# shadowk29/cusumtools

Hardware: NVIDIA B200
Metric: Msamples/s filtered+CUSUM-segmented (higher is better)
Workload: dtype f32

## Files before the change

cusumtools_b200/csrc/ct_detect.cu:

```cuda
#include "ct_common.cuh"
#include "cusumtools_b200.h"

namespace {

constexpr int kRun = 4096;
constexpr int kRunWords = kRun / 32;
constexpr int kDetWarps = 8;

struct RunSummary {
    unsigned first_last;
    unsigned ns0;
    unsigned ne0;
    unsigned pad;
};

__device__ __forceinline__ unsigned automaton_word(unsigned A, unsigned B, unsigned& c) {
    unsigned P = ~(A | B);
    unsigned long long X = (unsigned long long)(A | P), Y = (unsigned long long)A;
    unsigned long long sum = X + Y + c;
    unsigned long long cin = sum ^ X ^ Y;
    unsigned I = (unsigned)(cin >> 1);
    c = I >> 31;
    return I;
}
// ... 95 lines not shown
        A[2 * k] = A[2 * k + 1] = a; B[2 * k] = B[2 * k + 1] = b;
        mixed[k] = mix;
    }
#pragma unroll
    for (int k = 0; k < 2; ++k) {
        unsigned todo = __ballot_sync(CT_FULL, mixed[k]);
        while (todo) {
            const int src = __ffs(todo) - 1;
            todo &= todo - 1;
            const long long p0 = base + (2 * src + k) * 64 + lane, p1 = p0 + 32;
            const float v0 = p0 < n ? sgn * y[p0] : te, v1 = p1 < n ? sgn * y[p1] : te;
            const unsigned a0 = __ballot_sync(CT_FULL, v0 < ts), b0 = __ballot_sync(CT_FULL, v0 > te);
            const unsigned a1 = __ballot_sync(CT_FULL, v1 < ts), b1 = __ballot_sync(CT_FULL, v1 > te);
            if (lane == src) { A[2 * k] = a0; B[2 * k] = b0; A[2 * k + 1] = a1; B[2 * k + 1] = b1; }
        }
    }
    uint4* mout = reinterpret_cast<uint4*>(masks + run * kRunWords + 4 * lane);
    mout[0] = make_uint4(A[0], B[0], A[1], B[1]);
    mout[1] = make_uint4(A[2], B[2], A[3], B[3]);
    unsigned lastIn = 0, firstIn = 0, any = 0;
#pragma unroll
    for (int w = 0; w < 4; ++w) {
        const unsigned nz = A[w] | B[w];
        if (nz) {
            if (!any) firstIn = (A[w] >> (__ffs(nz) - 1)) & 1u;
            lastIn = (A[w] >> (31 - __clz(nz))) & 1u;
            any = 1;
        }
    }
    const unsigned nzmask = __ballot_sync(CT_FULL, any != 0);
    const unsigned lastmask = __ballot_sync(CT_FULL, lastIn != 0);
    const unsigned firstmask = __ballot_sync(CT_FULL, firstIn != 0);
    const unsigned lower = nzmask & ((1u << lane) - 1u);
    unsigned c = lower ? ((lastmask >> (31 - __clz(lower))) & 1u) : 0u;
    unsigned ns = 0, ne = 0;
#pragma unroll
    for (int w = 0; w < 4; ++w) {
        const unsigned cprev = c;
        const unsigned I = automaton_word(A[w], B[w], c);
        const unsigned prev = (I << 1) | cprev;
        ns += __popc(I & ~prev);
        ne += __popc(~I & prev);
    }
#pragma unroll
    for (int o = 16; o > 0; o >>= 1) { ns += __shfl_xor_sync(CT_FULL, ns, o); ne += __shfl_xor_sync(CT_FULL, ne, o); }
    if (lane == 0) {
        unsigned first = 0, last = 0;
        if (nzmask) {
            first = ((firstmask >> (__ffs(nzmask) - 1)) & 1u) ? 1u : 2u;
            last = ((lastmask >> (31 - __clz(nzmask))) & 1u) ? 1u : 2u;
        }
        RunSummary s; s.first_last = first | (last << 2); s.ns0 = ns; s.ne0 = ne; s.pad = 0;
        summ[run] = s;
    }
}

__device__ __forceinline__ void adjusted(const RunSummary& s, unsigned st, unsigned& a, unsigned& b) {
    const unsigned f = s.first_last & 3;
    a = s.ns0; b = s.ne0;
    if (st == 1) { if (f == 1) a -= 1; else if (f == 2) b += 1; }
}
constexpr int kGroup = 64;
__global__ void ct_detect_scan_groups(const RunSummary* __restrict__ summ, long long nruns,
                                      RunSummary* __restrict__ gsum, long long ngroups) {
    const long long g = (long long)blockIdx.x * blockDim.x + threadIdx.x;
    if (g >= ngroups) return;
    const long long r0 = g * kGroup, r1 = (r0 + kGroup < nruns) ? r0 + kGroup : nruns;
    unsigned st = 2, first = 0, last = 0, ns = 0, ne = 0;
    for (long long r = r0; r < r1; ++r) {
        const RunSummary s = summ[r];
        unsigned a, b; adjusted(s, st, a, b);
        ns += a; ne += b;
        const unsigned f = s.first_last & 3, l = (s.first_last >> 2) & 3;
        if (!first) first = f;
        if (l) { last = l; st = l; }
    }
    RunSummary o; o.first_last = first | (last << 2); o.ns0 = ns; o.ne0 = ne; o.pad = 0;
    gsum[g] = o;
}
__global__ void ct_detect_scan_expand(const RunSummary* __restrict__ summ, long long nruns,
                                      const uint4* __restrict__ ginfo, const unsigned long long* __restrict__ goffs,
                                      long long ngroups, uint4* __restrict__ runinfo,
                                      unsigned long long* __restrict__ offs) {
    const long long g = (long long)blockIdx.x * blockDim.x + threadIdx.x;
    if (g >= ngroups) return;
    const long long r0 = g * kGroup, r1 = (r0 + kGroup < nruns) ? r0 + kGroup : nruns;
    unsigned st = ginfo[g].x ? 1u : 2u;
    unsigned long long ns = goffs[2 * g], ne = goffs[2 * g + 1];
    for (long long r = r0; r < r1; ++r) {
        const RunSummary s = summ[r];
        unsigned a, b; adjusted(s, st, a, b);
        runinfo[r] = make_uint4(st == 1 ? 1u : 0u, 0u, 0u, 0u);
        offs[2 * r] = ns; offs[2 * r + 1] = ne;
        ns += a; ne += b;
        const unsigned l = (s.first_last >> 2) & 3;
        if (l) st = l;
    }
}

__global__ void __launch_bounds__(1024)
ct_detect_scan(const RunSummary* __restrict__ summ, long long nruns, int state_in,
               uint4* __restrict__ runinfo ,
               unsigned long long* __restrict__ offs ,
               unsigned long long* __restrict__ counts ) {
    __shared__ unsigned s_last[1024];
    __shared__ unsigned long long s_ns[1024], s_ne[1024];
    __shared__ unsigned s_statein[1024];
    const int tid = threadIdx.x;
    const long long per = (nruns + 1023) / 1024;
    const long long r0 = tid * per, r1 = (r0 + per < nruns) ? r0 + per : nruns;
    unsigned last = 0;
    for (long long r = r0; r < r1; ++r) { unsigned l = (summ[r].first_last >> 2) & 3; if (l) last = l; }
    s_last[tid] = last;
    __syncthreads();
    if (tid == 0) {
        unsigned st = state_in ? 1u : 2u;
        for (int i = 0; i < 1024; ++i) { s_statein[i] = st; if (s_last[i]) st = s_last[i]; }
    }
    __syncthreads();
    unsigned st = s_statein[tid];
    unsigned long long ns = 0, ne = 0;
    for (long long r = r0; r < r1; ++r) {
        RunSummary s = summ[r];
        unsigned f = s.first_last & 3, l = (s.first_last >> 2) & 3;
        unsigned a = s.ns0, b = s.ne0;
        if (st == 1) { if (f == 1) a -= 1; else if (f == 2) b += 1; }
        ns += a; ne += b;
        if (l) st = l;
    }
    s_ns[tid] = ns; s_ne[tid] = ne;
    __syncthreads();
    if (tid == 0) {
        unsigned long long a = 0, b = 0;
        for (int i = 0; i < 1024; ++i) {
            unsigned long long ta = s_ns[i], tb = s_ne[i];
            s_ns[i] = a; s_ne[i] = b; a += ta; b += tb;
        }
        counts[0] = a; counts[1] = b;
    }
    __syncthreads();
    st = s_statein[tid]; ns = s_ns[tid]; ne = s_ne[tid];
    for (long long r = r0; r < r1; ++r) {
        RunSummary s = summ[r];
        unsigned f = s.first_last & 3, l = (s.first_last >> 2) & 3;
        unsigned a = s.ns0, b = s.ne0;
        if (st == 1) { if (f == 1) a -= 1; else if (f == 2) b += 1; }
        runinfo[r] = make_uint4(st == 1 ? 1u : 0u, 0u, 0u, 0u);
        offs[2 * r] = ns; offs[2 * r + 1] = ne;
        ns += a; ne += b;
        if (l) st = l;
    }
}

__global__ void __launch_bounds__(128)
ct_detect_pass2(const uint2* __restrict__ masks, const uint4* __restrict__ runinfo,
                const unsigned long long* __restrict__ offs, long long nruns,
                long long* __restrict__ starts, long long* __restrict__ ends, long long cap) {
    const long long run = (long long)blockIdx.x * blockDim.x + threadIdx.x;
    if (run >= nruns) return;
    unsigned c = runinfo[run].x;
    unsigned long long os = offs[2 * run], oe = offs[2 * run + 1];
    const uint4* m4 = reinterpret_cast<const uint4*>(masks + run * kRunWords);
    const long long base = run * kRun;
    for (int w = 0; w < kRunWords; w += 2) {
        uint4 q = m4[w >> 1];
        unsigned AB[2][2] = {{q.x, q.y}, {q.z, q.w}};
#pragma unroll
        for (int j = 0; j < 2; ++j) {
            unsigned A = AB[j][0], B = AB[j][1];
            if ((A | B) == 0) continue;
            unsigned cprev = c;
            unsigned I = automaton_word(A, B, c);
            unsigned prev = (I << 1) | cprev;
            unsigned S = I & ~prev, E = ~I & prev;
            const long long wb = base + (long long)(w + j) * 32;
            while (S) { int b = __ffs(S) - 1; S &= S - 1; if ((long long)os < cap) starts[os] = wb + b; ++os; }
            while (E) { int b = __ffs(E) - 1; E &= E - 1; if ((long long)oe < cap) ends[oe] = wb + b; ++oe; }
        }
    }
}

constexpr int kStatChunk = 8192;
__global__ void __launch_bounds__(256)
ct_block_stats_kernel(const float* __restrict__ y, long long n, long long block, long long chunks_per_block,
                      float bmin, float bmax, float c0, float scale,
                      long long* __restrict__ cnt, long long* __restrict__ s1, long long* __restrict__ s2) {
    const long long kb = blockIdx.x / chunks_per_block;
    const long long ch = blockIdx.x % chunks_per_block;
    const long long b0 = kb * block + ch * kStatChunk;
    long long b1 = b0 + kStatChunk;
    const long long bend = (kb + 1) * block < n ? (kb + 1) * block : n;
    if (b1 > bend) b1 = bend;
    const int lane = ct_lane();
    const unsigned half_mask = 0xffffu << (lane & 16);
    long long c = 0, a = 0, b = 0;
    const bool aligned = (reinterpret_cast<uintptr_t>(y + b0) & 15) == 0;
    for (long long wb = b0 + (long long)(threadIdx.x & ~31) * 4; wb < b1; wb += 1024) {
        const long long p0 = wb + lane * 4;
        float v[4] = {0.f, 0.f, 0.f, 0.f};
        int have = 0;
        if (aligned && p0 + 4 <= b1) {
            const uint4 q = ct_ldg_stream(y + p0);
            v[0] = __uint_as_float(q.x); v[1] = __uint_as_float(q.y); v[2] = __uint_as_float(q.z); v[3] = __uint_as_float(q.w);
            have = 4;
        } else {
#pragma unroll
            for (int e = 0; e < 4; ++e) if (p0 + e < b1) { v[e] = y[p0 + e]; have = e + 1; }
        }
        bool ok = true;
#pragma unroll
        for (int e = 0; e < 4; ++e) if (e < have) ok = ok && v[e] >= bmin && v[e] <= bmax;
        const unsigned votes = __ballot_sync(CT_FULL, ok);
        if ((votes & half_mask) == half_mask) {
#pragma unroll
            for (int e = 0; e < 4; ++e) {
                if (e < have) {
                    const long long q = (long long)__float2ll_rn(__fmul_rn(__fsub_rn(v[e], c0), scale));
                    c += 1; a += q; b += q * q;
                }
            }
        }
    }
#pragma unroll
    for (int o = 16; o > 0; o >>= 1) {
        c += __shfl_xor_sync(CT_FULL, c, o);
        a += __shfl_xor_sync(CT_FULL, a, o);
        b += __shfl_xor_sync(CT_FULL, b, o);
    }
    if (lane == 0 && c) {
        atomicAdd(reinterpret_cast<unsigned long long*>(cnt + kb), (unsigned long long)c);
        atomicAdd(reinterpret_cast<unsigned long long*>(s1 + kb), (unsigned long long)a);
        atomicAdd(reinterpret_cast<unsigned long long*>(s2 + kb), (unsigned long long)b);
    }
}


__global__ void __launch_bounds__(1024)
ct_baseline_finalize_kernel(const long long* __restrict__ cnt, const long long* __restrict__ s1,
                            const long long* __restrict__ s2, long long nb, double c0, double inv_sc,
                            long long min_count, double thr, double thr_end, double* __restrict__ mean,
                            double* __restrict__ sd, int* __restrict__ sign, float* __restrict__ t_start,
                            float* __restrict__ t_end, int* __restrict__ status) {
    __shared__ long long s_first;
    __shared__ long long s_warp_last[32], s_warp_first[32];
    for (long long k = threadIdx.x; k < nb; k += blockDim.x) {
        const long long c = cnt[k];
        double m = __longlong_as_double(0x7ff8000000000000LL), s = m;
        if (c >= min_count) {
            const double cd = (double)c;
            const double ma = __ddiv_rn((double)s1[k], cd);
            m = __dadd_rn(c0, __dmul_rn(ma, inv_sc));
            double var = __dsub_rn(__ddiv_rn((double)s2[k], cd), __dmul_rn(ma, ma));
            if (!(var > 0.0)) var = 0.0;
            s = __dmul_rn(__dsqrt_rn(var), inv_sc);
        }
        mean[k] = m; sd[k] = s;
    }
    __syncthreads();
    const int lane = threadIdx.x & 31, wid = threadIdx.x >> 5, nwarp = blockDim.x >> 5;
    const long long per = (nb + blockDim.x - 1) / blockDim.x;
    const long long lo = (long long)threadIdx.x * per, hi = lo + per < nb ? lo + per : nb;
    const long long kNone = 0x7fffffffffffffffLL;
    long long last = -1, first = kNone;
    for (long long k = lo; k < hi; ++k)
        if (cnt[k] >= min_count) { last = k; if (first == kNone) first = k; }
    long long inc = last, fmin = first;
#pragma unroll
    for (int d = 1; d < 32; d <<= 1) {
        const long long t = __shfl_up_sync(CT_FULL, inc, d);
        if (lane >= d && t > inc) inc = t;
        const long long u = __shfl_xor_sync(CT_FULL, fmin, d);
        if (u < fmin) fmin = u;
    }
    if (lane == 31) s_warp_last[wid] = inc;
    if (lane == 0) s_warp_first[wid] = fmin;
    __syncthreads();
    long long before = -1;
    for (int w = 0; w < wid; ++w) if (s_warp_last[w] > before) before = s_warp_last[w];
    long long prev = __shfl_up_sync(CT_FULL, inc, 1);
    if (lane == 0) prev = -1;
    if (before > prev) prev = before;
    if (threadIdx.x == 0) {
        long long f = kNone;
        for (int w = 0; w < nwarp; ++w) if (s_warp_first[w] < f) f = s_warp_first[w];
        s_first = f == kNone ? -1 : f;
        *status = f == kNone ? 1 : 0;
    }
    __syncthreads();
    if (s_first < 0) return;
    {
        long long run = prev >= 0 ? prev : s_first;
        double rm = mean[run], rs = sd[run];
        for (long long k = lo; k < hi; ++k) {
            if (cnt[k] >= min_count) { rm = mean[k]; rs = sd[k]; }
            else { mean[k] = rm; sd[k] = rs; }
        }
    }
    __syncthreads();
    if (s_first < 0) return;
    for (long long k = threadIdx.x; k < nb; k += blockDim.x) {
        const double m = mean[k], s = sd[k];
        const int sg = m >= 0.0 ? 1 : -1;
        sign[k] = sg;
        t_start[k] = __double2float_rn(__dsub_rn(m, __dmul_rn(sg > 0 ? thr : -thr, s)));
        t_end[k] = __double2float_rn(__dsub_rn(m, __dmul_rn(sg > 0 ? thr_end : -thr_end, s)));
    }
}

__global__ void ct_event_windows_kernel(const long long* __restrict__ starts, const long long* __restrict__ ends,
                                        const unsigned long long* __restrict__ counts2, long long capacity,
                                        long long n_total, long long pos_lo, long long pos_hi, long long padding,
                                        long long minpoints, long long maxpoints, long long* __restrict__ w0,
                                        long long* __restrict__ w1, int* __restrict__ type, long long* __restrict__ out2) {
    long long ne = (long long)min(counts2[0], counts2[1]);
    if (ne > capacity) ne = capacity;
    auto lower = [&](long long pos) {
        long long a = 0, b = ne;
        while (a < b) { const long long m = (a + b) >> 1; if (starts[m] < pos) a = m + 1; else b = m; }
        return a;
    };
    const long long i0 = lower(pos_lo), i1 = lower(pos_hi);
    const long long t0 = (long long)blockIdx.x * blockDim.x + threadIdx.x;
    const long long stride = (long long)gridDim.x * blockDim.x;
    if (t0 == 0) { out2[0] = i1 - i0; out2[1] = i0; }
    for (long long i = i0 + t0; i < i1; i += stride) {
        const long long s = starts[i], e = ends[i];
        const long long a = s - padding, b = e + padding, len = e - s;
        const long long prev_end = i > i0 ? ends[i - 1] : (i0 > 0 ? ends[i0 - 1] : 0);
        const long long next_start = i + 1 < ne ? starts[i + 1] : n_total;
        int t = 0;
        if (a < prev_end || b > next_start || a < 0 || b > n_total) t = 4;
        if (len > maxpoints) t = 3;
        if (len < minpoints) t = 2;
        w0[i - i0] = a; w1[i - i0] = b; type[i - i0] = t;
    }
}


__global__ void __launch_bounds__(256)
ct_intra_crossings_kernel(const float* __restrict__ y, long long ntot, const long long* __restrict__ w0,
                          const long long* __restrict__ w1, const long long* __restrict__ es, long long nev,
                          const long long* __restrict__ nev_dev, long long block, long long nblocks,
                          const int* __restrict__ sign, const float* __restrict__ ts, const float* __restrict__ te,
                          int K, int* __restrict__ count, int* __restrict__ pairs) {
    if (nev_dev) { const long long d = *nev_dev; nev = d < nev ? d : nev; }
    const int lane = ct_lane();
    const long long gw = ((long long)blockIdx.x * blockDim.x + threadIdx.x) >> 5;
    const long long nw = ((long long)gridDim.x * blockDim.x) >> 5;
    for (long long ev = gw; ev < nev; ev += nw) {
        long long a = w0[ev], b = w1[ev];
        const long long org = a;
        if (a < 0) a = 0;
        if (b > ntot) b = ntot;
        long long kb = es[ev] / block;
        if (kb < 0) kb = 0;
        if (kb >= nblocks) kb = nblocks - 1;
        const float sg = sign[kb] > 0 ? 1.f : -1.f;
        const float tst = sg * ts[kb], ten = sg * te[kb];
        unsigned c = 0;
        int cnt = 0;
        int* out = pairs + ev * 2 * (long long)K;
        for (long long p = a; p < b; p += 32) {
            const long long i = p + lane;
            const bool valid = i < b;
            const float v = valid ? sg * y[i] : 0.f;
            const unsigned A = __ballot_sync(CT_FULL, valid && v < tst);
            const unsigned B = __ballot_sync(CT_FULL, valid && v > ten);
            const unsigned before = c;
            const unsigned I = automaton_word(A, B, c);
            const unsigned prev = (I << 1) | before;
            unsigned m = (I & ~prev) | (~I & prev);
            if (lane == 0) {
                while (m) {
                    const int bit = __ffs(m) - 1;
                    m &= m - 1;
                    const int idx = (int)(p - org) + bit;
                    if ((I >> bit) & 1u) { if (cnt < K) out[2 * cnt] = idx; }
                    else { if (cnt < K) out[2 * cnt + 1] = idx; ++cnt; }
                }
            }
        }
        if (lane == 0) {
            if (c) { if (cnt < K) out[2 * cnt + 1] = (int)(b - org); ++cnt; }
            count[ev] = cnt;
        }
    }
}

}

extern "C" {

int ct_detect_run(void) { return kRun; }

int64_t ct_detect_workspace_bytes(int64_t n) {
    long long nruns = (n + kRun - 1) / kRun;
    if (nruns < 1) nruns = 1;
    auto al = [](long long b) { return (b + 255) / 256 * 256; };
    long long ng = (nruns + kGroup - 1) / kGroup;
    return al(nruns * kRunWords * 8) + al(nruns * 16) + al(nruns * 16) + al(nruns * 16) + 3 * al(ng * 16);
}

int ct_block_stats_f32(const float* y, int64_t n, int64_t block, float bmin, float bmax, float c0,
                       int shift, int64_t* cnt, int64_t* s1, int64_t* s2, void* stream) {
    if (!y || !cnt || !s1 || !s2 || n < 0 || block <= 0) { ct_set_error("block_stats: bad argument"); return CT_ERR_ARG; }
    if (block % 64) { ct_set_error("block_stats: the baseline block must be a multiple of 64 samples (the chunk of the in-window rule)"); return CT_ERR_ARG; }
    long long nb = (n + block - 1) / block;
    cudaStream_t st = (cudaStream_t)stream;
    if (nb == 0) return CT_OK;
    cudaMemsetAsync(cnt, 0, nb * 8, st); cudaMemsetAsync(s1, 0, nb * 8, st); cudaMemsetAsync(s2, 0, nb * 8, st);
    long long cpb = (block + kStatChunk - 1) / kStatChunk;
    long long grid = nb * cpb;
    if (grid > 0x7fffffffLL) { ct_set_error("block_stats: trace too long for one launch"); return CT_ERR_UNSUPPORTED; }
    CT_COUNT_LAUNCH();
    ct_block_stats_kernel<<<(unsigned)grid, 256, 0, st>>>(y, n, block, cpb, bmin, bmax, c0, ldexpf(1.f, shift), (long long*)cnt, (long long*)s1, (long long*)s2);
    return ct_check_launch("ct_block_stats_kernel");
}

int ct_detect_f32(const float* y, int64_t n, int64_t block, const int32_t* sign, const float* t_start,
                  const float* t_end, int state_in, const float* chunk_minmax, int64_t minmax_shift, void* workspace,
                  int64_t workspace_bytes, int64_t* starts, int64_t* ends, int64_t capacity, uint64_t* counts2, void* stream) {
    if (!y || !sign || !t_start || !t_end || !workspace || !starts || !ends || !counts2 || n < 0) {
        ct_set_error("detect: bad argument"); return CT_ERR_ARG;
    }
    if (block <= 0 || block % kRun) { ct_set_error("detect: baseline block must be a multiple of %d samples", kRun); return CT_ERR_ARG; }
    if (workspace_bytes < ct_detect_workspace_bytes(n)) { ct_set_error("detect: workspace too small"); return CT_ERR_ARG; }
    cudaStream_t st = (cudaStream_t)stream;
    if (n == 0) { cudaMemsetAsync(counts2, 0, 16, st); return CT_OK; }
    long long nruns = (n + kRun - 1) / kRun;
    auto al = [](long long b) { return (b + 255) / 256 * 256; };
    char* w = (char*)workspace;
    uint2* masks = (uint2*)w;            w += al(nruns * kRunWords * 8);
    RunSummary* summ = (RunSummary*)w;   w += al(nruns * 16);
    uint4* runinfo = (uint4*)w;          w += al(nruns * 16);
    unsigned long long* offs = (unsigned long long*)w;  w += al(nruns * 16);
    const long long ng = (nruns + kGroup - 1) / kGroup;
    RunSummary* gsum = (RunSummary*)w;   w += al(ng * 16);
    uint4* ginfo = (uint4*)w;            w += al(ng * 16);
    unsigned long long* goffs = (unsigned long long*)w;
    long long g1 = (nruns + kDetWarps - 1) / kDetWarps;
    if (chunk_minmax && (minmax_shift < 0 || minmax_shift % 64 || (reinterpret_cast<uintptr_t>(chunk_minmax) & 7))) {
        ct_set_error("detect: chunk extrema need an 8-byte aligned array and a shift that is a multiple of 64"); return CT_ERR_ARG;
    }
    CT_COUNT_LAUNCH();
    if (chunk_minmax)
        ct_detect_pass1_minmax<<<(unsigned)g1, kDetWarps * 32, 0, st>>>(y, n, block, sign, t_start, t_end,
                                                                        reinterpret_cast<const float2*>(chunk_minmax), minmax_shift,
                                                                        masks, summ, nruns);
    else
        ct_detect_pass1<<<(unsigned)g1, kDetWarps * 32, 0, st>>>(y, n, block, sign, t_start, t_end, masks, summ, nruns);
    int rc = ct_check_launch("ct_detect_pass1"); if (rc) return rc;
    CT_COUNT_LAUNCH();
    ct_detect_scan_groups<<<(unsigned)((ng + 127) / 128), 128, 0, st>>>(summ, nruns, gsum, ng);
    rc = ct_check_launch("ct_detect_scan_groups"); if (rc) return rc;
    CT_COUNT_LAUNCH();
    ct_detect_scan<<<1, 1024, 0, st>>>(gsum, ng, state_in, ginfo, goffs, (unsigned long long*)counts2);
    rc = ct_check_launch("ct_detect_scan"); if (rc) return rc;
    CT_COUNT_LAUNCH();
    ct_detect_scan_expand<<<(unsigned)((ng + 127) / 128), 128, 0, st>>>(summ, nruns, ginfo, goffs, ng, runinfo, offs);
    rc = ct_check_launch("ct_detect_scan_expand"); if (rc) return rc;
    CT_COUNT_LAUNCH();
    ct_detect_pass2<<<(unsigned)((nruns + 127) / 128), 128, 0, st>>>(masks, runinfo, offs, nruns, (long long*)starts, (long long*)ends, capacity);
    return ct_check_launch("ct_detect_pass2");
}

int ct_baseline_finalize(const int64_t* cnt, const int64_t* s1, const int64_t* s2, int64_t nb, float c0, int shift,
                         int64_t min_count, double threshold, double hysteresis, double* mean, double* stdev,
                         int32_t* sign, float* t_start, float* t_end, int32_t* status, void* stream) {
    if (!cnt || !s1 || !s2 || !mean || !stdev || !sign || !t_start || !t_end || !status || nb < 0) {
        ct_set_error("baseline_finalize: bad argument"); return CT_ERR_ARG;
    }
    if (nb == 0) return CT_OK;
    CT_COUNT_LAUNCH();
    ct_baseline_finalize_kernel<<<1, 1024, 0, (cudaStream_t)stream>>>(
        (const long long*)cnt, (const long long*)s1, (const long long*)s2, nb, (double)c0, ldexp(1.0, -shift), min_count,
        threshold, threshold - hysteresis, mean, stdev, sign, t_start, t_end, status);
    return ct_check_launch("ct_baseline_finalize_kernel");
}

int ct_event_windows(const int64_t* starts, const int64_t* ends, const uint64_t* counts2, int64_t capacity,
                     int64_t n_total, int64_t pos_lo, int64_t pos_hi, int64_t padding, int64_t minpoints, int64_t maxpoints,
                     int64_t* win_start, int64_t* win_end, int32_t* type, int64_t* out2, void* stream) {
    if (!starts || !ends || !counts2 || !win_start || !win_end || !type || !out2 || capacity < 0) {
        ct_set_error("event_windows: bad argument"); return CT_ERR_ARG;
    }
    cudaStream_t st = (cudaStream_t)stream;
    cudaMemsetAsync(out2, 0, 16, st);
    if (capacity == 0) return CT_OK;
    long long grid = (capacity + 255) / 256;
    const long long cap = (long long)ct_sm_count() * 8;
    if (grid > cap) grid = cap;
    CT_COUNT_LAUNCH();
    ct_event_windows_kernel<<<(unsigned)grid, 256, 0, st>>>(
        (const long long*)starts, (const long long*)ends, (const unsigned long long*)counts2, capacity, n_total, pos_lo, pos_hi,
        padding, minpoints, maxpoints, (long long*)win_start, (long long*)win_end, type, (long long*)out2);
    return ct_check_launch("ct_event_windows_kernel");
}

int ct_intra_crossings_f32(const float* y, int64_t n_total, const int64_t* win_start, const int64_t* win_end,
                           const int64_t* ev_start, int64_t n_events, const int64_t* n_events_dev, int64_t block,
                           int64_t n_blocks, const int32_t* sign, const float* t_start, const float* t_end,
                           int32_t max_pairs, int32_t* count, int32_t* pairs, void* stream) {
    if (!y || !win_start || !win_end || !ev_start || !sign || !t_start || !t_end || !count || !pairs || n_events < 0) {
        ct_set_error("intra_crossings: bad argument"); return CT_ERR_ARG;
    }
    if (block <= 0 || n_blocks <= 0 || max_pairs < 1) { ct_set_error("intra_crossings: need block > 0, n_blocks > 0, max_pairs >= 1"); return CT_ERR_ARG; }
    if (n_events == 0) return CT_OK;
    long long grid = (n_events + 7) / 8;
    const long long cap = (long long)ct_sm_count() * 8;
    if (grid > cap) grid = cap;
    CT_COUNT_LAUNCH();
    ct_intra_crossings_kernel<<<(unsigned)grid, 256, 0, (cudaStream_t)stream>>>(
        y, n_total, (const long long*)win_start, (const long long*)win_end, (const long long*)ev_start, n_events,
        (const long long*)n_events_dev, block, n_blocks, sign, t_start, t_end, max_pairs, count, pairs);
    return ct_check_launch("ct_intra_crossings_kernel");
}


}
```

cusumtools_b200/csrc/ct_cusum.cu:

```cuda
#include "ct_common.cuh"
#include "cusumtools_b200.h"

namespace {

constexpr int kE = 8;
constexpr int kBlk = 32 * kE;
constexpr float kQ = 64.0f, kSScale = 1024.0f, kSMax = 2097152.0f;
constexpr int kBig = 0x3fffffff;

struct CusumArgs {
    const float* y; long long ntot;
    const long long* w0; const long long* w1; const int* type; long long nev;
    const long long* nev_dev;
    float delta, h; int max_levels;
    int* n_levels; int* edges; double* mean; double* sd; unsigned char* overflow;
    unsigned long long* counter;
    int* pending;
    const int* order;
};

__device__ __forceinline__ void warp_excl_add2(int v, long long w, int lane, int& exv, long long& exw, int& totv,
                                               long long& totw) {
    int iv = v; long long iw = w;
#pragma unroll
// ... 92 lines not shown
#pragma unroll
                    for (int e = 0; e < kE; ++e) xv[e] = xn[e];
                } else {
                    load_block(rs, xv);
                }
                if (rs + kBlk < n) { load_block(rs + kBlk, xn); pref_rs = rs + kBlk; }
#pragma unroll
                for (int e = 0; e < kE; ++e) q[e] = quantise(xv[e], x0);
            }
            int pq[kE]; long long pqq[kE];
            {
                int aq = 0; long long aqq = 0;
#pragma unroll
                for (int e = 0; e < kE; ++e) {
                    const int k = r0 + e;
                    const int qv = (k >= k0 && k < n) ? q[e] - qa : 0;
                    aq += qv; aqq += (long long)qv * qv;
                    pq[e] = aq; pqq[e] = aqq;
                }
            }
            int totq, exq; long long totqq, exqq;
            warp_excl_add2(pq[kE - 1], pqq[kE - 1], lane, exq, exqq, totq, totqq);
            int lp[kE], ln[kE];
            {
                int ap = 0, an = 0;
#pragma unroll
                for (int e = 0; e < kE; ++e) {
                    const int k = r0 + e;
                    int sp = 0, sn = 0;
                    if (k > k0 && k < n) {
                        const int cnt = k - k0 + 1;
                        const float rc = __fdiv_rn(1.0f, (float)cnt);
                        const float m = cusum_mean(cSq + exq + pq[e], rc);
                        const float t = __fsub_rn((float)(q[e] - qa), m);
                        const SeqOut o = cusum_tail(cSqq + exqq + pqq[e], m, rc, t, dq, hq);
                        sp = o.sp; sn = o.sn;
                    }
                    ap += sp; an += sn;
                    lp[e] = ap; ln[e] = an;
                }
            }
            int lmp = kBig, lmn = kBig;
#pragma unroll
            for (int e = 0; e < kE; ++e) { lmp = min(lmp, lp[e]); lmn = min(lmn, ln[e]); }
            int totp, totn, bminp, bminn, exp_, exn_, exmp, exmn;
            warp_excl_summin2(lp[kE - 1], lmp, ln[kE - 1], lmn, lane, exp_, exmp, exn_, exmn, totp, bminp, totn, bminn);
#pragma unroll
            for (int e = 0; e < kE; ++e) { lp[e] += exp_; ln[e] += exn_; }
            exmp = min(exmp, mp); exmn = min(exmn, mn);
            int firste = kE, zp = -1, zn = -1;
            int gpd[kE], gnd[kE];
            {
                int rp = exmp, rn = exmn;
#pragma unroll
                for (int e = 0; e < kE; ++e) {
                    const int k = r0 + e;
                    rp = min(rp, lp[e]); rn = min(rn, ln[e]);
                    gpd[e] = lp[e] - rp; gnd[e] = ln[e] - rn;
                    const bool valid = k > k0 && k < n;
                    if (valid && firste == kE && (gpd[e] > H || gnd[e] > H)) firste = e;
                }
            }
            const unsigned hit = __ballot_sync(CT_FULL, firste < kE);
            int limit = min(rs + kBlk, n) - 1;
            int kdet = -1, gp_d = 0, gn_d = 0;
            if (hit) {
                const int ld = __ffs(hit) - 1;
                const int ef = __shfl_sync(CT_FULL, firste, ld);
                kdet = rs + ld * kE + ef;
                int mygp = 0, mygn = 0;
#pragma unroll
                for (int e = 0; e < kE; ++e) if (e == ef) { mygp = gpd[e]; mygn = gnd[e]; }
                gp_d = __shfl_sync(CT_FULL, mygp, ld);
                gn_d = __shfl_sync(CT_FULL, mygn, ld);
                limit = kdet;
            }
#pragma unroll
            for (int e = 0; e < kE; ++e) {
                const int k = r0 + e;
                if (k >= k0 && k <= limit) { if (gpd[e] == 0) zp = k; if (gnd[e] == 0) zn = k; }
            }
            zp = warp_max(zp); zn = warp_max(zn);
            if (zp >= 0) argp = zp;
            if (zn >= 0) argn = zn;
            if (hit) {
                const int jmin = (gp_d >= gn_d) ? argp : argn;
                if (nedge >= a.max_levels) { overflow = 1; break; }
                if (lane == 0) ed[nedge] = jmin + 1;
                ++nedge;
                k0 = kdet; cSq = 0; cSqq = 0; mp = kBig; mn = kBig; argp = kdet; argn = kdet;
                qa = quantise(a.y[p0 + kdet], x0);
                const int nrs = rs + ((kdet - rs) & ~(kE - 1));
                fresh = nrs != rs;
                rs = nrs;
            } else {
                cSq += totq; cSqq += totqq;
                const long long nmp = (long long)min(mp, bminp) - totp, nmn = (long long)min(mn, bminn) - totn;
                mp = (int)max(min(nmp, (long long)kBig), -(long long)kBig);
                mn = (int)max(min(nmn, (long long)kBig), -(long long)kBig);
                rs += kBlk;
                fresh = true;
            }
        }
        if (lane == 0) { ed[nedge] = n; a.n_levels[ev] = nedge; a.overflow[ev] = (unsigned char)overflow; }
        __syncwarp();
        for (int i = 0; i < nedge; ++i) {
            const int e0 = ed[i], e1 = ed[i + 1];
            long long sq = 0, sqq = 0;
            for (int k = e0 + lane; k < e1; k += 32) {
                const long long qv = quantise(a.y[p0 + k], x0);
                sq += qv; sqq += qv * qv;
            }
#pragma unroll
            for (int o = 16; o > 0; o >>= 1) { sq += __shfl_xor_sync(CT_FULL, sq, o); sqq += __shfl_xor_sync(CT_FULL, sqq, o); }
            if (lane == 0) {
                const double len = (double)(e1 - e0), ad = (double)sq, bd = (double)sqq;
                a.mean[ev * a.max_levels + i] = __dadd_rn((double)x0, __ddiv_rn(__ddiv_rn(ad, len), 64.0));
                double var = __dsub_rn(bd, __ddiv_rn(__dmul_rn(ad, ad), len));
                if (var < 0.0) var = 0.0;
                a.sd[ev * a.max_levels + i] = __ddiv_rn(__dsqrt_rn(__ddiv_rn(var, len)), 64.0);
            }
        }
        __syncwarp();
    }
}

__global__ void __launch_bounds__(128, 4) ct_cusum_warp_kernel(CusumArgs a) {
    const int lane = ct_lane();
    const int H = __float2int_rn(__fmul_rn(a.h, kSScale));
    const float dq = __fmul_rn(a.delta, kQ);
    const float hq = __fmul_rn(dq, 0.5f);
    const bool aligned = (reinterpret_cast<uintptr_t>(a.y) & 31) == 0;
    const unsigned long long npend = a.counter[1];
    for (;;) {
        unsigned long long i = 0;
        if (lane == 0) i = atomicAdd(a.counter + 2, 1ULL);
        i = __shfl_sync(CT_FULL, i, 0);
        if (i >= npend) break;
        warp_event(a, (long long)a.pending[i], lane, H, dq, hq, aligned);
        __syncwarp();
    }
}

constexpr int kS = 8;
constexpr int kPiece = 32;
constexpr int kRowB = 144;
constexpr int kStageB = 32 * kRowB;
constexpr int kStages = 2;
#ifndef CT_CUSUM_SEQ_WARPS
#define CT_CUSUM_SEQ_WARPS 20
#endif
constexpr int kSeqWarps = CT_CUSUM_SEQ_WARPS;
constexpr int kSeqMax = 16384;
constexpr int kSeqTab = 8192 + 16;
constexpr int kSeqTabLead = 8;
constexpr int kSeqSmem = (kSeqTab + kSeqTabLead) * 4 + kSeqWarps * kStages * kStageB;
constexpr int kSeqMinEvents = 16384;
constexpr unsigned char kRawSums = 0x80;

__device__ __forceinline__ void level_sums(long long Sd, long long Sdd, int cnt, int qa, long long& Sq, long long& Sqq) {
    Sq = Sd + (long long)cnt * qa;
    Sqq = Sdd + 2LL * qa * Sd + (long long)cnt * ((long long)qa * qa);
}
__device__ __forceinline__ void cp_async16(unsigned dst, const void* src, int bytes) {
    asm volatile("cp.async.cg.shared.global [%0], [%1], 16, %2;" :: "r"(dst), "l"(src), "r"(bytes) : "memory");
}

__global__ void __launch_bounds__(kSeqWarps * 32, 1) ct_cusum_seq_kernel(CusumArgs a) {
    extern __shared__ __align__(128) unsigned char smem[];
    float* rct = reinterpret_cast<float*>(smem) + kSeqTabLead;
    const int lane = ct_lane();
    unsigned char* wbuf = smem + (kSeqTab + kSeqTabLead) * 4 + (threadIdx.x >> 5) * (kStages * kStageB);
    for (int i = (int)threadIdx.x - kSeqTabLead; i < kSeqTab; i += blockDim.x) rct[i] = i > 0 ? __fdiv_rn(1.0f, (float)i) : 0.f;
    __syncthreads();
    const int H = __float2int_rn(__fmul_rn(a.h, kSScale));
    const float dq = __fmul_rn(a.delta, kQ);
    const float hq = __fmul_rn(dq, 0.5f);
    long long nev = a.nev;
    if (a.nev_dev) { const long long d = *a.nev_dev; nev = d < nev ? d : nev; }
    const int ML = a.max_levels;
    const bool aligned = (reinterpret_cast<uintptr_t>(a.y) & 15) == 0;
    const long long seq_limit = (nev < kSeqMinEvents || !aligned) ? 0 : kSeqMax;
    const long long full_lines = a.ntot >> 5;

    bool exhausted = false;
    int f_ev = 0, f_n = 0, f_kb = 0, f_left = 0;
    unsigned f_line = 0;
    auto fetch = [&](int stage) {
        unsigned need = __ballot_sync(CT_FULL, f_left == 0 && !exhausted);
        while (need) {
            const int leader = __ffs(need) - 1;
            long long base = 0;
            if (lane == leader) base = (long long)atomicAdd(a.counter, (unsigned long long)__popc(need));
            base = __shfl_sync(CT_FULL, base, leader);
            if (f_left == 0 && !exhausted) {
                const long long slot = base + __popc(need & ((1u << lane) - 1u));
                if (slot >= nev) exhausted = true;
                else {
                    const long long ev = a.order ? a.order[slot] : slot;
                    const long long p0 = a.w0[ev];
                    const long long nn = a.w1[ev] - p0;
                    const bool bad = nn <= 0 || p0 < 0 || a.w1[ev] > a.ntot || nn > 0x3fffffffLL || (a.type && a.type[ev] != 0);
                    if (bad) { a.n_levels[ev] = 0; a.overflow[ev] = 0; }
                    else if (nn > seq_limit) a.pending[atomicAdd(a.counter + 1, 1ULL)] = (int)ev;
                    else {
                        f_ev = (int)ev; f_n = (int)nn;
                        f_kb = -(int)(p0 & (kPiece - 1));
                        f_line = (unsigned)(p0 >> 5);
                        f_left = (f_n - f_kb + kPiece - 1) >> 5;
                        a.edges[ev * (ML + 1)] = 0;
                    }
                }
            }
            need = __ballot_sync(CT_FULL, f_left == 0 && !exhausted);
        }
        unsigned char* st = wbuf + stage * kStageB;
        const bool has = f_left > 0;
        *reinterpret_cast<int4*>(st + lane * kRowB + 128) = make_int4(has ? f_ev : -1, f_kb, f_n, (int)f_line);
        int avail = 0;
        if (has) avail = (long long)f_line < full_lines ? kPiece : (int)(a.ntot - ((long long)f_line << 5));
        const unsigned myline = has ? f_line : 0u;
        const unsigned dst0 = (unsigned)__cvta_generic_to_shared(st) + (lane >> 3) * kRowB + (lane & 7) * 16;
        const char* src0 = reinterpret_cast<const char*>(a.y) + (lane & 7) * 16;
        const int c4 = (lane & 7) * 4;
        if (__all_sync(CT_FULL, avail == kPiece)) {
#pragma unroll
            for (int it = 0; it < 8; ++it) {
                const unsigned L = __shfl_sync(CT_FULL, myline, it * 4 + (lane >> 3));
                cp_async16(dst0 + it * 4 * kRowB, src0 + ((unsigned long long)L << 7), 16);
            }
        } else {
#pragma unroll
            for (int it = 0; it < 8; ++it) {
                const unsigned L = __shfl_sync(CT_FULL, myline, it * 4 + (lane >> 3));
                const int A = __shfl_sync(CT_FULL, avail, it * 4 + (lane >> 3));
                cp_async16(dst0 + it * 4 * kRowB, src0 + ((unsigned long long)L << 7), min(max(A - c4, 0), 4) * 4);
            }
        }
        asm volatile("cp.async.commit_group;" ::: "memory");
        if (has) { ++f_line; f_kb += kPiece; --f_left; }
    };

    bool running = false;
    long long p0 = 0;
    int ev = 0, n = 0;
    float x0 = 0.f, nx0 = 0.f;
    int k0 = 0, qa = 0, gp = 0, gn = 0, rp = 0, rn = 0, nedge = 1, e0 = 0;
    long long Sd = 0, Sdd = 0;
    long long Lp = 0, Lpp = 0;
    long long ZpS = 0, ZpSS = 0, ZnS = 0, ZnSS = 0;

#pragma unroll
    for (int s = 0; s < kStages; ++s) fetch(s);
    int stage = 0;
    for (;;) {
        asm volatile("cp.async.wait_group %0;" :: "n"(kStages - 1) : "memory");
        __syncwarp();
        const float* row = reinterpret_cast<const float*>(wbuf + stage * kStageB + lane * kRowB);
        const int4 hdr = *reinterpret_cast<const int4*>(row + kPiece);
        const bool hev = hdr.x >= 0;
        if (__ballot_sync(CT_FULL, hev) == 0) break;
        const int kb = hdr.y;
        if (hev && kb <= 0) {
            ev = hdr.x; n = hdr.z;
            p0 = ((long long)(unsigned)hdr.w << 5) - kb;
            x0 = row[-kb];
            nx0 = __fmul_rn(x0, -kQ);
            k0 = 0; qa = 0; gp = gn = 0; rp = rn = 0; nedge = 1; e0 = 0;
            Sd = Sdd = 0; Lp = Lpp = 0;
            running = true;
        }
#pragma unroll 1
        for (int g = 0; g < kPiece / kS; ++g) {
            const int gk = kb + g * kS;
            const bool act = hev && running && gk < n && gk + kS > 0;
            if (!__any_sync(CT_FULL, act)) continue;
            float xv[kS];
            {
                const float4 u = *reinterpret_cast<const float4*>(row + g * kS);
                const float4 v = *reinterpret_cast<const float4*>(row + g * kS + 4);
                xv[0] = u.x; xv[1] = u.y; xv[2] = u.z; xv[3] = u.w; xv[4] = v.x; xv[5] = v.y; xv[6] = v.z; xv[7] = v.w;
            }
            unsigned nlim = act ? (unsigned)n : 0u;
            if (__any_sync(CT_FULL, act && gk < 0)) {
#pragma unroll
                for (int e = 0; e < kS - 1; ++e)
                    if (gk + e < 0) xv[e] = x0;
            }
            const int endc = n - gk;
            int dv[kS];
            int s32 = (int)Sd;
            unsigned nq = 0;
            {
                const bool att = act && (gp | gn) == 0 && gk - k0 + kS < kSeqTab &&
                                 (unsigned long long)(Sd + (1LL << 30)) < (1ULL << 31);
                const float* rcp = rct + (att ? gk - k0 + 1 : 1);
#pragma unroll
                for (int e = 0; e < kS; ++e) {
                    dv[e] = __float2int_rn(__fmaf_rn(xv[e], kQ, nx0)) - qa;
                    s32 += dv[e];
                    const float t = __fsub_rn((float)dv[e], __fmul_rn(__int2float_rn(s32), rcp[e]));
                    if (!(fabsf(t) <= hq)) nq |= 1u << e;
                }
                if (endc < kS) nq &= (1u << endc) - 1u;
                nq |= 1u << kS;
                if (!att) nq = 1u;
                if (!act) nq = 1u << kS;
            }
            const int F = (int)__reduce_min_sync(CT_FULL, (unsigned)(__ffs(nq) - 1));
            if (F > 0 && act) {
                if (F == kS && endc >= kS) {
                    Sd = s32;
#pragma unroll
                    for (int e = 0; e < kS; ++e) Sdd += (long long)dv[e] * dv[e];
                } else {
                    const int lim = min(F, endc);
#pragma unroll
                    for (int e = 0; e < kS; ++e)
                        if (e < lim) { Sd += dv[e]; Sdd += (long long)dv[e] * dv[e]; }
                }
                rp = rn = max(gk + F - 1, 0);
            }
            if (F < kS) {
#pragma unroll 1
            for (int e = F; e < kS; ++e) {
                const int k = gk + e;
                const bool valid = (unsigned)k < nlim;
                const int q = __float2int_rn(__fmaf_rn(row[g * kS + e], kQ, nx0));
                const int d = valid ? q - qa : 0;
                Sd += d; Sdd += (long long)d * d;
                const int cnt = valid ? k - k0 + 1 : 1;
                float rc = rct[min(cnt, kSeqTab - 1)];
                if (cnt >= kSeqTab) rc = __fdiv_rn(1.0f, (float)cnt);
                const float m = cusum_mean(Sd, rc);
                const float t = __fsub_rn((float)d, m);
                const bool quiet = !valid || ((gp | gn) == 0 && fabsf(t) <= hq);
                if (__all_sync(CT_FULL, quiet)) { if (valid) { rp = k; rn = k; } continue; }
                const SeqOut s = cusum_tail(Sdd, m, rc, t, dq, hq);
                if (!valid) continue;
                if (gp == 0) { ZpS = Sd - d; ZpSS = Sdd - (long long)d * d; }
                if (gn == 0) { ZnS = Sd - d; ZnSS = Sdd - (long long)d * d; }
                gp = max(gp + s.sp, 0); rp = gp == 0 ? k : rp;
                gn = max(gn + s.sn, 0); rn = gn == 0 ? k : rn;
                if (max(gp, gn) > H) {
                    if (nedge >= ML) {
                        long long T = 0, TT = 0;
#pragma unroll 1
                        for (int j = e0; j < n; ++j) { const long long qj = quantise(a.y[p0 + j], x0); T += qj; TT += qj * qj; }
                        const long long r_ = (long long)ev * ML + (nedge - 1);
                        reinterpret_cast<long long*>(a.mean)[r_] = T;
                        reinterpret_cast<long long*>(a.sd)[r_] = TT;
                        a.edges[(long long)ev * (ML + 1) + nedge] = n;
                        a.n_levels[ev] = nedge;
                        a.overflow[ev] = (unsigned char)(1 | kRawSums);
                        running = false; nlim = 0u;
                        continue;
                    }
                    const bool pwin = gp >= gn;
                    const int edge = (pwin ? rp : rn) + 1;
                    const long long zs = pwin ? ZpS : ZnS, zss = pwin ? ZpSS : ZnSS;
                    long long Aq, Aqq, Bq, Bqq;
                    level_sums(zs, zss, edge - k0, qa, Aq, Aqq);
                    level_sums(Sd - zs - d, Sdd - zss - (long long)d * d, k - edge, qa, Bq, Bqq);
                    const long long r_ = (long long)ev * ML + (nedge - 1);
                    CT_CHECK_RANGE(r_, 1, a.nev * ML, "cusum, level row");
                    reinterpret_cast<long long*>(a.mean)[r_] = Lp + Aq;
                    reinterpret_cast<long long*>(a.sd)[r_] = Lpp + Aqq;
                    a.edges[(long long)ev * (ML + 1) + nedge] = edge;
                    ++nedge;
                    e0 = edge; Lp = Bq; Lpp = Bqq;
                    k0 = k; qa = q; Sd = 0; Sdd = 0; gp = gn = 0; rp = rn = k;
                }
            }
            }
            if (act && running && gk + kS >= n) {
                long long Sq, Sqq;
                level_sums(Sd, Sdd, n - k0, qa, Sq, Sqq);
                const long long r_ = (long long)ev * ML + (nedge - 1);
                reinterpret_cast<long long*>(a.mean)[r_] = Lp + Sq;
                reinterpret_cast<long long*>(a.sd)[r_] = Lpp + Sqq;
                a.edges[(long long)ev * (ML + 1) + nedge] = n;
                a.n_levels[ev] = nedge;
                a.overflow[ev] = kRawSums;
                running = false;
            }
        }
        __syncwarp();
        fetch(stage);
        stage = stage + 1 == kStages ? 0 : stage + 1;
    }
    asm volatile("cp.async.wait_group 0;" ::: "memory");
}

constexpr int kLenClasses = 64;
__device__ __forceinline__ int len_class(long long len) {
    if (len <= 0 || len > kSeqMax) return 0;
    const int c = (int)((len - 1) >> 8);
    return kLenClasses - 1 - (c < kLenClasses - 2 ? c : kLenClasses - 2);
}
__global__ void __launch_bounds__(256) ct_cusum_order_count(const long long* __restrict__ w0, const long long* __restrict__ w1,
                                                             long long nev, const long long* __restrict__ nev_dev,
                                                             unsigned* __restrict__ cls_count) {
    __shared__ unsigned h[kLenClasses];
    if (nev_dev) { const long long d = *nev_dev; nev = d < nev ? d : nev; }
    if (threadIdx.x < kLenClasses) h[threadIdx.x] = 0;
    __syncthreads();
    for (long long ev = (long long)blockIdx.x * blockDim.x + threadIdx.x; ev < nev; ev += (long long)gridDim.x * blockDim.x)
        atomicAdd(&h[len_class(w1[ev] - w0[ev])], 1u);
    __syncthreads();
    if (threadIdx.x < kLenClasses && h[threadIdx.x]) atomicAdd(&cls_count[threadIdx.x], h[threadIdx.x]);
}
__global__ void __launch_bounds__(256) ct_cusum_order_fill(const long long* __restrict__ w0, const long long* __restrict__ w1,
                                                            long long nev, const long long* __restrict__ nev_dev,
                                                            const unsigned* __restrict__ cls_count, unsigned* __restrict__ cls_fill,
                                                            int* __restrict__ order) {
    __shared__ unsigned base[kLenClasses], h[kLenClasses], off[kLenClasses];
    if (nev_dev) { const long long d = *nev_dev; nev = d < nev ? d : nev; }
    if (threadIdx.x == 0) {
        unsigned acc = 0;
        for (int c = 0; c < kLenClasses; ++c) { base[c] = acc; acc += cls_count[c]; }
    }
    constexpr int kChunk = 256 * 16;
    for (long long c0 = (long long)blockIdx.x * kChunk; c0 < nev; c0 += (long long)gridDim.x * kChunk) {
        __syncthreads();
        if (threadIdx.x < kLenClasses) h[threadIdx.x] = 0;
        __syncthreads();
        int cls[16]; unsigned pos[16];
#pragma unroll
        for (int i = 0; i < 16; ++i) {
            const long long ev = c0 + i * 256 + threadIdx.x;
            cls[i] = -1;
            if (ev < nev) { cls[i] = len_class(w1[ev] - w0[ev]); pos[i] = atomicAdd(&h[cls[i]], 1u); }
        }
        __syncthreads();
        if (threadIdx.x < kLenClasses && h[threadIdx.x]) off[threadIdx.x] = base[threadIdx.x] + atomicAdd(&cls_fill[threadIdx.x], h[threadIdx.x]);
        __syncthreads();
#pragma unroll
        for (int i = 0; i < 16; ++i)
            if (cls[i] >= 0) {
                CT_CHECK_RANGE(off[cls[i]] + pos[i], 1, nev, "cusum, hand-out order");
                order[off[cls[i]] + pos[i]] = (int)(c0 + i * 256 + threadIdx.x);
            }
    }
}

__device__ __forceinline__ void finalize_level(const CusumArgs& a, long long i, double x0, int e0, int e1) {
    const double len = (double)(e1 - e0);
    const double ad = (double)reinterpret_cast<const long long*>(a.mean)[i];
    const double bd = (double)reinterpret_cast<const long long*>(a.sd)[i];
    a.mean[i] = __dadd_rn(x0, __ddiv_rn(__ddiv_rn(ad, len), 64.0));
    double var = __dsub_rn(bd, __ddiv_rn(__dmul_rn(ad, ad), len));
    if (var < 0.0) var = 0.0;
    a.sd[i] = __ddiv_rn(__dsqrt_rn(__ddiv_rn(var, len)), 64.0);
}
__global__ void ct_cusum_finalize_kernel(CusumArgs a) {
    long long nev = a.nev;
    if (a.nev_dev) { const long long d = *a.nev_dev; nev = d < nev ? d : nev; }
    const int ML = a.max_levels;
    for (long long ev = (long long)blockIdx.x * blockDim.x + threadIdx.x; ev < nev; ev += (long long)gridDim.x * blockDim.x) {
        const unsigned char f = a.overflow[ev];
        if (!(f & kRawSums)) continue;
        const int* ed = a.edges + ev * (ML + 1);
        const int nl = a.n_levels[ev];
        const double x0 = (double)a.y[a.w0[ev]];
        for (int lv = 0; lv < nl; ++lv) finalize_level(a, ev * ML + lv, x0, ed[lv], ed[lv + 1]);
        a.overflow[ev] = f & (unsigned char)~kRawSums;
    }
}
__global__ void __launch_bounds__(256) ct_cusum_finalize_rows_kernel(CusumArgs a) {
    long long nev = a.nev;
    if (a.nev_dev) { const long long d = *a.nev_dev; nev = d < nev ? d : nev; }
    const int ML = a.max_levels;
    const long long total = nev * ML;
    const long long stride = (long long)gridDim.x * blockDim.x;
    for (long long i0 = (long long)blockIdx.x * blockDim.x; i0 < total; i0 += stride) {
        const long long i = i0 + threadIdx.x;
        const bool in = i < total;
        const long long ev = in ? i / ML : 0;
        const int lv = (int)(i - ev * ML);
        unsigned char f = 0;
        int nl = 0;
        if (in) { f = a.overflow[ev]; nl = a.n_levels[ev]; }
        const bool raw = in && (f & kRawSums);
        if (raw && lv < nl) {
            const int* ed = a.edges + ev * (ML + 1);
            finalize_level(a, i, (double)a.y[a.w0[ev]], ed[lv], ed[lv + 1]);
// ... 201 lines not shown
```

Measured before the change: 311,000.

## Parallelize detect pass2 across a warp per run with ballot carry and scan

Pass2 used to give each 4096-sample run to a single thread, which walked 128 mask words serially. Now a warp owns a run and each lane handles 4 words. Each lane's carry-in comes from a ballot over the last nonzero input bit of lower lanes, and a warp shuffle-up prefix sum of start/end popcounts gives every lane its output offset. This removes the long serial dependency per thread and makes the mask loads coalesced, at the cost of a warp-level scan and a launch grid that relies on g1 matching the run count.

```diff
diff --git a/cusumtools_b200/csrc/ct_detect.cu b/cusumtools_b200/csrc/ct_detect.cu
--- a/cusumtools_b200/csrc/ct_detect.cu
+++ b/cusumtools_b200/csrc/ct_detect.cu
@@ -271,31 +271,51 @@
     }
 }
 
-__global__ void __launch_bounds__(128)
+__global__ void __launch_bounds__(kDetWarps * 32)
 ct_detect_pass2(const uint2* __restrict__ masks, const uint4* __restrict__ runinfo,
                 const unsigned long long* __restrict__ offs, long long nruns,
                 long long* __restrict__ starts, long long* __restrict__ ends, long long cap) {
-    const long long run = (long long)blockIdx.x * blockDim.x + threadIdx.x;
+    const int lane = ct_lane();
+    const long long run = (long long)blockIdx.x * kDetWarps + (threadIdx.x >> 5);
     if (run >= nruns) return;
-    unsigned c = runinfo[run].x;
-    unsigned long long os = offs[2 * run], oe = offs[2 * run + 1];
-    const uint4* m4 = reinterpret_cast<const uint4*>(masks + run * kRunWords);
+    const uint4* m4 = reinterpret_cast<const uint4*>(masks + run * kRunWords + 4 * lane);
+    const uint4 q0 = m4[0], q1 = m4[1];
+    unsigned A[4] = {q0.x, q0.z, q1.x, q1.z}, B[4] = {q0.y, q0.w, q1.y, q1.w};
+    unsigned lastIn = 0, any = 0;
+#pragma unroll
+    for (int w = 0; w < 4; ++w) {
+        const unsigned nz = A[w] | B[w];
+        if (nz) { lastIn = (A[w] >> (31 - __clz(nz))) & 1u; any = 1; }
+    }
+    const unsigned nzmask = __ballot_sync(CT_FULL, any != 0);
+    const unsigned lastmask = __ballot_sync(CT_FULL, lastIn != 0);
+    const unsigned lower = nzmask & ((1u << lane) - 1u);
+    unsigned c = lower ? ((lastmask >> (31 - __clz(lower))) & 1u) : runinfo[run].x;
+    unsigned cs = 0, ce = 0;
+#pragma unroll
+    for (int w = 0; w < 4; ++w) {
+        const unsigned cprev = c;
+        const unsigned I = automaton_word(A[w], B[w], c);
+        const unsigned prev = (I << 1) | cprev;
+        A[w] = I & ~prev;
+        B[w] = ~I & prev;
+        cs += __popc(A[w]);
+        ce += __popc(B[w]);
+    }
+    unsigned xs = cs, xe = ce;
+#pragma unroll
+    for (int d = 1; d < 32; d <<= 1) {
+        const unsigned us = __shfl_up_sync(CT_FULL, xs, d), ue = __shfl_up_sync(CT_FULL, xe, d);
+        if (lane >= d) { xs += us; xe += ue; }
+    }
+    unsigned long long os = offs[2 * run] + (xs - cs), oe = offs[2 * run + 1] + (xe - ce);
     const long long base = run * kRun;
-    for (int w = 0; w < kRunWords; w += 2) {
-        uint4 q = m4[w >> 1];
-        unsigned AB[2][2] = {{q.x, q.y}, {q.z, q.w}};
-#pragma unroll
-        for (int j = 0; j < 2; ++j) {
-            unsigned A = AB[j][0], B = AB[j][1];
-            if ((A | B) == 0) continue;
-            unsigned cprev = c;
-            unsigned I = automaton_word(A, B, c);
-            unsigned prev = (I << 1) | cprev;
-            unsigned S = I & ~prev, E = ~I & prev;
-            const long long wb = base + (long long)(w + j) * 32;
-            while (S) { int b = __ffs(S) - 1; S &= S - 1; if ((long long)os < cap) starts[os] = wb + b; ++os; }
-            while (E) { int b = __ffs(E) - 1; E &= E - 1; if ((long long)oe < cap) ends[oe] = wb + b; ++oe; }
-        }
+#pragma unroll
+    for (int w = 0; w < 4; ++w) {
+        const long long wb = base + (4 * lane + w) * 32;
+        unsigned S = A[w], E = B[w];
+        while (S) { const int b = __ffs(S) - 1; S &= S - 1; if (os < (unsigned long long)cap) starts[os] = wb + b; ++os; }
+        while (E) { const int b = __ffs(E) - 1; E &= E - 1; if (oe < (unsigned long long)cap) ends[oe] = wb + b; ++oe; }
     }
 }
 
@@ -579,7 +599,7 @@
     ct_detect_scan_expand<<<(unsigned)((ng + 127) / 128), 128, 0, st>>>(summ, nruns, ginfo, goffs, ng, runinfo, offs);
     rc = ct_check_launch("ct_detect_scan_expand"); if (rc) return rc;
     CT_COUNT_LAUNCH();
-    ct_detect_pass2<<<(unsigned)((nruns + 127) / 128), 128, 0, st>>>(masks, runinfo, offs, nruns, (long long*)starts, (long long*)ends, capacity);
+    ct_detect_pass2<<<(unsigned)g1, kDetWarps * 32, 0, st>>>(masks, runinfo, offs, nruns, (long long*)starts, (long long*)ends, capacity);
     return ct_check_launch("ct_detect_pass2");
 }
 
```

Result: no change. 313,800 (median of 6 runs) (+0.9%).

## Replace per-sample quiet test with range-bound block test in CUSUM fast path

Applied to the files above, without the earlier changes.

The per-sample running-mean quiet check in the 8-sample fast path is replaced by a conservative bound. The mean is computed once at the block start, and the code checks that the spread of deviations around it stays within a margin derived from the threshold. Squared sums are accumulated in 32-bit around that mean and reconstructed algebraically, and a prefix fallback finds the first sample that can fail. This removes the per-sample reciprocal-table loads and float multiplies. The shared-memory table size is now derived from the warp count, and __fdiv_rn is swapped for __frcp_rn. The bound is more conservative than the old check, so more blocks may drop to the slow scalar path, and the unsigned wraparound arithmetic must stay exact.

```diff
diff --git a/cusumtools_b200/csrc/ct_cusum.cu b/cusumtools_b200/csrc/ct_cusum.cu
--- a/cusumtools_b200/csrc/ct_cusum.cu
+++ b/cusumtools_b200/csrc/ct_cusum.cu
@@ -268,8 +268,11 @@
 #endif
 constexpr int kSeqWarps = CT_CUSUM_SEQ_WARPS;
 constexpr int kSeqMax = 16384;
-constexpr int kSeqTab = 8192 + 16;
 constexpr int kSeqTabLead = 8;
+constexpr int kSmemMax = 227 * 1024;
+constexpr int kSeqTabFit = (kSmemMax - kSeqWarps * kStages * kStageB) / 4 - kSeqTabLead;
+constexpr int kSeqTab = kSeqTabFit < 8192 + 16 ? kSeqTabFit : 8192 + 16;
+static_assert(kSeqTab >= 1024, "too many warps for the shared memory");
 constexpr int kSeqSmem = (kSeqTab + kSeqTabLead) * 4 + kSeqWarps * kStages * kStageB;
 constexpr int kSeqMinEvents = 16384;
 constexpr unsigned char kRawSums = 0x80;
@@ -292,6 +295,7 @@
     const int H = __float2int_rn(__fmul_rn(a.h, kSScale));
     const float dq = __fmul_rn(a.delta, kQ);
     const float hq = __fmul_rn(dq, 0.5f);
+    const int hqi = hq >= 16383.f ? 16383 : (int)hq;
     long long nev = a.nev;
     if (a.nev_dev) { const long long d = *a.nev_dev; nev = d < nev ? d : nev; }
     const int ML = a.max_levels;
@@ -404,36 +408,52 @@
                     if (gk + e < 0) xv[e] = x0;
             }
             const int endc = n - gk;
-            int dv[kS];
-            int s32 = (int)Sd;
-            unsigned nq = 0;
+            int tv[kS];
+            int mi, st = 0;
+            unsigned stt = 0, Fl = kS;
             {
-                const bool att = act && (gp | gn) == 0 && gk - k0 + kS < kSeqTab &&
-                                 (unsigned long long)(Sd + (1LL << 30)) < (1ULL << 31);
-                const float* rcp = rct + (att ? gk - k0 + 1 : 1);
+                const int cp = gk - k0;
+                bool att = act && (gp | gn) == 0 && (unsigned long long)(Sd + (1LL << 30)) < (1ULL << 31);
+                float rcp = rct[att ? min(cp, kSeqTab - 1) : 0];
+                if (att && cp >= kSeqTab) rcp = __frcp_rn((float)cp);
+                mi = __float2int_rn(__fmul_rn(__int2float_rn(att ? (int)Sd : 0), rcp));
+                const unsigned am = (unsigned)abs(mi);
+                const int err = (int)(am >> 21) + 2;
+                const int B = hqi - 1 - (int)((am + (unsigned)err + (unsigned)hqi) >> 21);
+                att = att && B >= 0;
+                const int qc = qa + mi;
+                int lo = -err, hi = err;
 #pragma unroll
                 for (int e = 0; e < kS; ++e) {
-                    dv[e] = __float2int_rn(__fmaf_rn(xv[e], kQ, nx0)) - qa;
-                    s32 += dv[e];
-                    const float t = __fsub_rn((float)dv[e], __fmul_rn(__int2float_rn(s32), rcp[e]));
-                    if (!(fabsf(t) <= hq)) nq |= 1u << e;
+                    tv[e] = __float2int_rn(__fmaf_rn(xv[e], kQ, nx0)) - qc;
+                    lo = min(lo, tv[e]); hi = max(hi, tv[e]);
+                    st += tv[e];
+                    stt += (unsigned)tv[e] * (unsigned)tv[e];
                 }
-                if (endc < kS) nq &= (1u << endc) - 1u;
-                nq |= 1u << kS;
-                if (!att) nq = 1u;
-                if (!act) nq = 1u << kS;
-            }
-            const int F = (int)__reduce_min_sync(CT_FULL, (unsigned)(__ffs(nq) - 1));
+                const bool pass = att && (unsigned)(hi - lo) <= (unsigned)B;
+                if (act && !pass) Fl = 0;
+                if (__any_sync(CT_FULL, att && !pass)) {
+                    if (att && !pass) {
+                        lo = -err; hi = err;
+#pragma unroll
+                        for (int e = 0; e < kS; ++e) {
+                            if (e < endc) { lo = min(lo, tv[e]); hi = max(hi, tv[e]); }
+                            Fl += (unsigned)(hi - lo) <= (unsigned)B;
+                        }
+                    }
+                }
+            }
+            const int F = (int)__reduce_min_sync(CT_FULL, Fl);
             if (F > 0 && act) {
                 if (F == kS && endc >= kS) {
-                    Sd = s32;
-#pragma unroll
-                    for (int e = 0; e < kS; ++e) Sdd += (long long)dv[e] * dv[e];
+                    Sd += (long long)st + (long long)kS * mi;
+                    Sdd = (long long)((unsigned long long)Sdd + stt + 2ULL * (unsigned long long)((long long)mi * st) +
+                                      (unsigned long long)kS * (unsigned long long)((long long)mi * mi));
                 } else {
                     const int lim = min(F, endc);
 #pragma unroll
                     for (int e = 0; e < kS; ++e)
-                        if (e < lim) { Sd += dv[e]; Sdd += (long long)dv[e] * dv[e]; }
+                        if (e < lim) { const int d = tv[e] + mi; Sd += d; Sdd += (long long)d * d; }
                 }
                 rp = rn = max(gk + F - 1, 0);
             }
@@ -447,7 +467,7 @@
                 Sd += d; Sdd += (long long)d * d;
                 const int cnt = valid ? k - k0 + 1 : 1;
                 float rc = rct[min(cnt, kSeqTab - 1)];
-                if (cnt >= kSeqTab) rc = __fdiv_rn(1.0f, (float)cnt);
+                if (cnt >= kSeqTab) rc = __frcp_rn((float)cnt);
                 const float m = cusum_mean(Sd, rc);
                 const float t = __fsub_rn((float)d, m);
                 const bool quiet = !valid || ((gp | gn) == 0 && fabsf(t) <= hq);
```

Result: no change. 317,100 before, 316,900 after, median of 6 (-0.1%).
